# willSapgreen/stereo-vision

Measured on AMD Instinct MI355X. Metric: stereo pairs/sec (ELAS 1242x375, ROBOTICS, D1+D2+LR), higher is better.
Workload: dtype u8

## Files before the change

### include/svh.h

```cpp
#ifndef SVH_H
#define SVH_H

#include <stddef.h>
#include <stdint.h>

#ifdef __cplusplus
extern "C" {
#endif

#define SVH_OK                 0
#define SVH_ERR_FEW_SUPPORT    1
#define SVH_ERR_BAD_ARG       -1
#define SVH_ERR_HIP           -2
#define SVH_ERR_UNSUPPORTED   -3
#define SVH_ERR_NO_DEVICE     -4
#define SVH_ERR_BAD_DIMS      -7

typedef struct svh_elas_params {
    int32_t disp_min;
    int32_t disp_max;
    float   support_threshold;
    int32_t support_texture;
    int32_t candidate_stepsize;
    int32_t incon_window_size;
// ... 92 lines not shown
typedef struct svh_elas_stream svh_elas_stream;
svh_elas_stream* svh_elas_stream_open(svh_elas* e, const int32_t* dims, int32_t depth);
int32_t svh_elas_stream_push(svh_elas_stream* s, const uint8_t* I1, const uint8_t* I2,
                             float* D1, float* D2, uint64_t* ticket);
int32_t svh_elas_stream_push_device(svh_elas_stream* s, const uint8_t* dI1, const uint8_t* dI2,
                                    float* dD1, float* dD2, uint64_t* ticket);
int32_t svh_elas_stream_flush(svh_elas_stream* s);
int32_t svh_elas_stream_pop(svh_elas_stream* s, uint64_t* ticket, int32_t* status, int32_t timeout_ms);
int32_t svh_elas_stream_close(svh_elas_stream* s);
int32_t svh_elas_stream_push_device_n(svh_elas_stream* s, int32_t n, const uint8_t* dI1, const uint8_t* dI2,
                                      size_t in_stride, float* dD1, float* dD2, size_t out_stride,
                                      uint64_t* first_ticket);
int32_t svh_elas_stream_pop_n(svh_elas_stream* s, int32_t n, int32_t* status, int32_t* popped);
int32_t svh_elas_stream_push_n(svh_elas_stream* s, int32_t n, const uint8_t* const* I1, const uint8_t* const* I2,
                               float* const* D1, float* const* D2, uint64_t* first_ticket);

int64_t svh_elas_trim(void);

int32_t svh_elas_set_lanes(int32_t lanes);
int32_t svh_elas_set_group(int32_t pairs);

int32_t svh_elas_set_stage(int32_t where);
void svh_elas_stage_stats(int64_t* device_groups, int64_t* handed_back);
void svh_elas_get_settings(int32_t out[4]);

enum svh_elas_stage {
    SVH_ELAS_DESC1 = 0,
    SVH_ELAS_DESC2,
    SVH_ELAS_DCAN_RAW,
    SVH_ELAS_SUPPORT,
    SVH_ELAS_TRI1,
    SVH_ELAS_TRI2,
    SVH_ELAS_PLANES1,
    SVH_ELAS_PLANES2,
    SVH_ELAS_GRID1,
    SVH_ELAS_GRID2,
    SVH_ELAS_D1_RAW,
    SVH_ELAS_D2_RAW,
    SVH_ELAS_D1_LR,
    SVH_ELAS_D2_LR,
    SVH_ELAS_D1_SEG,
    SVH_ELAS_D2_SEG,
    SVH_ELAS_D1_GAP,
    SVH_ELAS_D2_GAP,
    SVH_ELAS_STAGE_COUNT
};
// ... 175 lines not shown
```

### stereo-vision_amd/csrc/elas_engine.cpp

```cpp
#include <hip/hip_runtime.h>
#include <stdio.h>
#include <string.h>

#include <atomic>
#include <chrono>
#include <condition_variable>
#include <deque>
#include <functional>
#include <algorithm>
#include <map>
#include <memory>
#include <mutex>
#include <string>
#include <thread>
#include <vector>

#include "hip_guard.h"
#include "svh_internal.h"

namespace svh {

static thread_local int t_device = 0;

#define HIP_TRY(kind, expr) SVH_HIP_TRY(nullptr, kind, expr)
// ... 72 lines not shown
    EventProfiler prof;
    int device = 0;
    hipStream_t stream = nullptr;
    hipEvent_t wait_ev = nullptr;
    hipStream_t copy_stream = nullptr;
    hipEvent_t match_ev = nullptr, copy_ev = nullptr;
    bool poll_wait = false;
    bool parallel_host = true;
    bool lone_group = true;
    int32_t W = 0, H = 0, disp_max = -1, step = 0, grid_size = 0, sub = -1, gcap = 0;
    Dims d{};
    bool desc_fly = false;
    int64_t owner_hi = 0;
    size_t prior_cap = 0;
    size_t ntri_max = 0;
    std::vector<HostPrior> hp;
    std::vector<int32_t> P;
    StageDev stg{};
    bool stage_ok = false;
    hipEvent_t stage_ev = nullptr;
    bool resident = false;
    bool force_host = false;
    float P_key[5] = {-1, -1, -1, -1, -1};
    size_t o_P = 0, o_sup = 0, o_tri = 0;

    void release() {
        if (!stream) return;
        (void)hipSetDevice(device);
        static_cast<LaneBufs&>(*this) = LaneBufs();
        stage_ok = false; stg = StageDev{};
        P_key[0] = -1;
        W = H = 0;
    }

    void destroy() {
        if (!stream) return;
        (void)hipSetDevice(device);
        release();
        for (hipEvent_t* e : {&wait_ev, &match_ev, &copy_ev, &stage_ev})
            if (*e) {
                (void)hipEventDestroy(*e);
                *e = nullptr;
            }
        for (hipEvent_t e : prof.ev) (void)hipEventDestroy(e);
        prof.ev.clear();
        prof.names.clear();
        if (copy_stream) (void)hipStreamDestroy(copy_stream);
        (void)hipStreamDestroy(stream);
        copy_stream = stream = nullptr;
    }

    int ensure(const svh_elas_params& p, int32_t w, int32_t h, int32_t g) {
        if (!stream) {
            HIP_TRY(none, hipSetDevice(device));
// ... 256 lines not shown
        if (!g_hostprof || !g_hp_pairs) return;
        static const char* nm[HP_N] = {"enqueue A", "waits", "filters", "delaunay", "pack", "enqueue B"};
        double tot = 0;
        for (int i = 0; i < HP_N; i++) tot += g_hp_ns[i];
        fprintf(stderr, "[svh host prof] %llu pairs, %.1f us cpu/pair:", (unsigned long long)g_hp_pairs.load(),
                tot / 1e3 / g_hp_pairs);
        for (int i = 0; i < HP_N; i++) fprintf(stderr, "  %s %.1f", nm[i], g_hp_ns[i] / 1e3 / g_hp_pairs);
        fprintf(stderr, "\n");
    }
};
static HostProfDump g_hp_dump;
#define HP_MARK(slot) do { if (g_hostprof) { uint64_t n_ = cpu_ns(); g_hp_ns[slot] += n_ - hp_t; hp_t = n_; } } while (0)

static int stage_mode_from_env() {
    const char* e = svh::env("SVH_STAGE");
    if (!e || !*e || !strcmp(e, "auto") || !strcmp(e, "-1")) return -1;
    if (!strcmp(e, "host") || !strcmp(e, "0")) return 0;
    if (!strcmp(e, "device") || !strcmp(e, "1")) return 1;
    fprintf(stderr, "svhip: SVH_STAGE=%s is not one of auto|-1, host|0, device|1: using auto\n", e);
    return -1;
}

static std::atomic<int64_t> g_stage_dev_groups{0}, g_stage_redo_groups{0};

static hipError_t event_wait(Lane& L, hipEvent_t ev) {
    if (!L.poll_wait || g_wait_us <= 0) return hipEventSynchronize(ev);
    for (;;) {
        hipError_t e = hipEventQuery(ev);
        if (e != hipErrorNotReady) return e;
        std::this_thread::sleep_for(std::chrono::microseconds(g_wait_us.load(std::memory_order_relaxed)));
    }
}

static int run_group_body(Lane& L, const svh_elas_params& p, const int32_t* dims, const GroupIO& io,
                          int32_t* status, Taps* taps, svh_elas* timing, int mode, int prefer_device);

static int run_group(Lane& L, const svh_elas_params& p, const int32_t* dims, const GroupIO& io,
                     int32_t* status, Taps* taps, svh_elas* timing, int mode = RG_ALL, int prefer_device = 0) {
    const int rc = run_group_body(L, p, dims, io, status, taps, timing, mode, prefer_device);
    if (rc == SVH_ERR_HIP) {
        const std::string keep = svh_last_error();
        if (L.stream) (void)hipStreamSynchronize(L.stream);
        if (L.copy_stream) (void)hipStreamSynchronize(L.copy_stream);
        (void)hipGetLastError();
        L.prof.used = 0;
        L.resident = false;
// ... 15 lines not shown
    if (rc) return rc;
    if (g > 1) taps = nullptr;
    const Dims& d = L.d;
    hipStream_t s = L.stream;
    L.prof.stream = s;
    const LaunchCtx cx = {s, g_prof_on.load() ? &L.prof : nullptr, L.lone_group};
    const size_t N = (size_t)W * H, DN = (size_t)d.DW * d.DH;
    const size_t nc = (size_t)d.Wc * d.Hc;
    const bool tapping = taps && taps->enabled;
    double t0 = now_ms();
    uint64_t hp_t = g_hostprof ? cpu_ns() : 0;

    GroupHdr* hdr = reinterpret_cast<GroupHdr*>(L.h_prior.p);
    DevMaps out;
    if (io.out_device) {
        out.D[0] = io.dD[0]; out.D[1] = io.dD[1]; out.stride[0] = out.stride[1] = io.out_stride;
    } else {
        out.D[0] = L.D; out.D[1] = L.D + DN; out.stride[0] = out.stride[1] = 2 * DN;
    }
    bool early_d2 = false;
    int32_t plane_radius = 2;

    auto enqueue_phase_b = [&](size_t o_P, size_t o_sup, size_t o_tri, int32_t total_sup, int32_t total_tri,
                               int32_t tri_bound) -> int {
        GroupDev G;
        G.hdr = reinterpret_cast<const GroupHdr*>(L.prior_dev.p);
        G.P = reinterpret_cast<const int32_t*>(L.prior_dev + o_P);
        G.support = reinterpret_cast<const int32_t*>(L.prior_dev + o_sup);
        G.tri = reinterpret_cast<const int32_t*>(L.prior_dev + o_tri);
        G.raster = L.raster;
        G.planes = L.planes;
        G.seed = L.seed;
        G.mask = L.mask;
        G.lists = L.lists;
        G.desc = L.desc;
        G.desc_fly = L.desc_fly ? 1 : 0;
        G.owner = L.owner;
        if (L.owner_hi + 1 + tri_bound >= INT32_MAX) {
            HIP_TRY(copy, hipMemsetAsync(L.owner, 0, (size_t)2 * L.gcap * N * sizeof(int32_t), s));
            L.owner_hi = 0;
        }
        G.owner_base = (int32_t)L.owner_hi;
        L.owner_hi += 1 + tri_bound;
        G.Draw = L.Draw;
        G.plane_radius = plane_radius;
        G.prior_absmax = 0;
        for (int32_t dd = 0; dd <= plane_radius && dd < (int32_t)L.P.size(); dd++)
            G.prior_absmax = std::max(G.prior_absmax, (int32_t)std::min<int64_t>(std::llabs((long long)L.P[dd]), INT32_MAX));
        launch_prior(cx, p, d, g, total_sup, total_tri, G);
        if (tapping) {
            const int32_t n1 = hdr->tri_end[0], n2 = hdr->tri_end[1] - hdr->tri_end[0];
            rc = tap_dev(L, taps, SVH_ELAS_PLANES1, L.planes.p, (size_t)6 * n1); if (rc) return rc;
            rc = tap_dev(L, taps, SVH_ELAS_PLANES2, L.planes.p + (size_t)6 * n1, (size_t)6 * n2); if (rc) return rc;
            const size_t words = (size_t)d.gw * d.gh * d.gwords;
            std::vector<uint32_t> m(2 * words);
            HIP_TRY(copy, hipMemcpyAsync(m.data(), L.mask, m.size() * sizeof(uint32_t), hipMemcpyDeviceToHost, s));
            HIP_TRY(wait, lane_wait(L));
            for (int k = 0; k < 2; k++) {
                std::vector<int32_t> gr;
                expand_grid(p, d, m.data() + k * words, gr);
                tap_host(taps, SVH_ELAS_GRID1 + k, gr.data(), gr.size());
            }
        }
        launch_owner(cx, p, d, g, total_tri, G);
        const bool tiles = !tapping && post_tiles_ok(p);
        const char* match_err = nullptr;
        const bool lr_done = launch_match(cx, p, d, g, G, &out, tapping, &match_err);
        if (match_err) return fail(SVH_ERR_HIP, std::string("launch_match: ") + match_err);
        early_d2 = !io.out_device && lr_done && !tapping && p.postprocess_only_left;
        if (early_d2) {
            if (!L.copy_stream) {
                HIP_TRY(none, hipStreamCreateWithFlags(&L.copy_stream, hipStreamNonBlocking));
                HIP_TRY(none, hipEventCreateWithFlags(&L.match_ev, hipEventDisableTiming));
                HIP_TRY(none, hipEventCreateWithFlags(&L.copy_ev, hipEventDisableTiming));
            }
            HIP_TRY(none, hipEventRecord(L.match_ev, s));
        }
        if (tapping) {
            rc = tap_dev(L, taps, SVH_ELAS_D1_RAW, L.Draw.p, DN); if (rc) return rc;
            rc = tap_dev(L, taps, SVH_ELAS_D2_RAW, L.Draw.p + DN, DN); if (rc) return rc;
        }
        const PostScratch ps = {L.tmp, L.labels, L.counts, L.seg_nroots};
        const int nside = p.postprocess_only_left ? 1 : 2;
        if (!lr_done) launch_lr(cx, p, d, g, G, out);
        if (tapping) {
            rc = tap_dev(L, taps, SVH_ELAS_D1_LR, out.D[0], DN); if (rc) return rc;
            rc = tap_dev(L, taps, SVH_ELAS_D2_LR, out.D[1], DN); if (rc) return rc;
// ... 42 lines not shown
            HIP_TRY(none, hipStreamWaitEvent(L.copy_stream, L.match_ev, 0));
            rc = copy_map(1, L.copy_stream, active);
            if (rc) return rc;
            HIP_TRY(none, hipEventRecord(L.copy_ev, L.copy_stream));
        }
        for (int k = 0; k < (early_d2 ? 1 : 2); k++) {
            rc = copy_map(k, s, active);
            if (rc) return rc;
        }
        if (early_d2) HIP_TRY(none, hipStreamWaitEvent(s, L.copy_ev, 0));
        return SVH_OK;
    };
    auto active_of = [&](int32_t j) {
        return L.h_counts.p->nsup[j] >= 3 && !(L.h_counts.p->flags[j] & (STG_DUP | STG_OVERFLOW));
    };

    auto finish = [&]() -> int {
        HIP_TRY(wait, lane_wait(L));
        HIP_TRY(launch, hipGetLastError());
        L.prof.collect();
        HP_MARK(HP_WAIT);
        if (!L.resident) return SVH_OK;
        g_stage_dev_groups++;
        bool redo = false;
        for (int32_t j = 0; j < g; j++) redo = redo || (L.h_counts.p->flags[j] & (STG_DUP | STG_OVERFLOW)) != 0;
        if (redo) {
            g_stage_redo_groups++;
            L.resident = false;
            L.force_host = true;
            rc = run_group(L, p, dims, io, status, taps, timing, RG_ALL, 0);
            L.force_host = false;
            return rc;
        }
        for (int32_t j = 0; j < g; j++) {
            if (L.h_counts.p->nsup[j] < 3) {
                printf("ERROR: Need at least 3 support points!\n");
                fflush(stdout);
                status[j] = SVH_ERR_FEW_SUPPORT;
            } else {
                status[j] = SVH_OK;
            }
        }
        return SVH_OK;
    };
    if (mode == RG_FINISH) return finish();

// ... 64 lines not shown
        L.resident = !L.force_host && L.stage_ok &&
                     (sm == 1 || (sm < 0 && prefer_device && stage_device_preferred(p, d, prefer_device > 1)));
        if (L.resident && prefer_device) L.poll_wait = true;
        if (!L.resident || tapping)
            HIP_TRY(copy, hipMemcpyAsync(L.h_dcan, L.dcan, g * nc * sizeof(int16_t), hipMemcpyDeviceToHost, s));
        if (L.resident) {
            prior_table(p, L.P, &plane_radius);
            const float key[5] = {p.beta, p.gamma, p.sigma, p.sradius, (float)p.disp_max};
            if (memcmp(key, L.P_key, sizeof(key)) != 0) {
                memcpy(L.h_prior + L.o_P, L.P.data(), L.P.size() * sizeof(int32_t));
                HIP_TRY(copy, hipMemcpyAsync(L.prior_dev + L.o_P, L.h_prior + L.o_P, L.P.size() * sizeof(int32_t),
                                       hipMemcpyHostToDevice, s));
                HIP_TRY(wait, hipStreamSynchronize(s));
                memcpy(L.P_key, key, sizeof(key));
            }
            if (tapping) {
                HIP_TRY(wait, hipStreamSynchronize(s));
                if (!L.desc_fly) {
                    rc = tap_dev(L, taps, SVH_ELAS_DESC1, L.desc.p, N * 16); if (rc) return rc;
                    rc = tap_dev(L, taps, SVH_ELAS_DESC2, L.desc.p + N * 16, N * 16); if (rc) return rc;
                }
                tap_host(taps, SVH_ELAS_DCAN_RAW, L.h_dcan.p, nc);
            }
            launch_stage_device(cx, p, d, g, L.stg, reinterpret_cast<GroupHdr*>(L.prior_dev.p),
                                reinterpret_cast<int32_t*>(L.prior_dev + L.o_sup),
                                reinterpret_cast<int32_t*>(L.prior_dev + L.o_tri));
            if (!L.stage_ev) HIP_TRY(none, hipEventCreateWithFlags(&L.stage_ev, hipEventDisableTiming));
            HIP_TRY(copy, hipMemcpyAsync(L.h_counts, L.stg.counts, sizeof(StageCounts), hipMemcpyDeviceToHost, s));
            HIP_TRY(none, hipEventRecord(L.stage_ev, s));
            if (tapping) {
                HIP_TRY(copy, hipMemcpyAsync(hdr, L.prior_dev, sizeof(GroupHdr), hipMemcpyDeviceToHost, s));
                HIP_TRY(wait, hipStreamSynchronize(s));
                if (hdr->active[0]) {
                    rc = tap_dev(L, taps, SVH_ELAS_SUPPORT, reinterpret_cast<int32_t*>(L.prior_dev + L.o_sup),
                                 (size_t)3 * hdr->total_sup); if (rc) return rc;
                    rc = tap_dev(L, taps, SVH_ELAS_TRI1, reinterpret_cast<int32_t*>(L.prior_dev + L.o_tri),
                                 (size_t)3 * hdr->tri_end[0]); if (rc) return rc;
                    rc = tap_dev(L, taps, SVH_ELAS_TRI2,
                                 reinterpret_cast<int32_t*>(L.prior_dev + L.o_tri) + (size_t)3 * hdr->tri_end[0],
                                 (size_t)3 * (hdr->tri_end[1] - hdr->tri_end[0])); if (rc) return rc;
                }
            }
            if (!tapping || hdr->active[0]) {
                const int32_t tri_bound = 2 * g * 2 * L.stg.sup_cap;
                rc = enqueue_phase_b(L.o_P, L.o_sup, L.o_tri, -1, -1, tri_bound);
                if (rc) return rc;
            }
        }
        HP_MARK(HP_ENQ_A);
    }
    if (!(mode & RG_HOST_B)) return SVH_OK;
    double t1 = t0, t2 = t0;
    if (L.resident) {
        if (!io.out_device) {
            HIP_TRY(wait, event_wait(L, L.stage_ev));
            HP_MARK(HP_WAIT);
            int32_t active[kMaxGroup];
            for (int32_t j = 0; j < g; j++) active[j] = active_of(j);
            rc = copy_out(active);
            if (rc) return rc;
        }
        if (g_hostprof) g_hp_pairs += g;
        HP_MARK(HP_ENQ_B);
        t1 = t2 = now_ms();
    } else {
    const bool warm = L.parallel_host && g == 1;
    if (warm) helpers_warm(3, 1500);
    struct WarmOff {
// ... 65 lines not shown
    const size_t o_sup = off;
    for (int32_t j = 0; j < g; j++) {
        const std::vector<int32_t>& v = L.hp[j].support;
        if (!v.empty()) memcpy(L.h_prior + off, v.data(), v.size() * sizeof(int32_t));
        off += v.size() * sizeof(int32_t);
    }
    off = (off + 63) & ~(size_t)63;
    const size_t o_tri = off;
    for (int32_t j = 0; j < g; j++)
        for (int k = 0; k < 2; k++) {
            const std::vector<int32_t>& v = L.hp[j].tri[k];
            if (!v.empty()) memcpy(L.h_prior + off, v.data(), v.size() * sizeof(int32_t));
            off += v.size() * sizeof(int32_t);
        }
    if (off > L.prior_cap) return fail(SVH_ERR_BAD_ARG, "prior exceeds staging capacity");
    if (warm_off.on) {
        helpers_warm(0, 0);
        warm_off.on = false;
    }
    t2 = now_ms();
    HP_MARK(HP_PACK);

    HIP_TRY(copy, hipMemcpyAsync(L.prior_dev, L.h_prior, off, hipMemcpyHostToDevice, s));
    rc = enqueue_phase_b(o_P, o_sup, o_tri, total_sup, total_tri, total_tri);
    if (rc) return rc;
    rc = copy_out(hdr->active);
    if (rc) return rc;
    HP_MARK(HP_ENQ_B);
    }
    if (!(mode & RG_FINISH)) return SVH_OK;
    rc = finish();
    if (rc) return rc;
    double t3 = now_ms();
    if (timing) {
        timing->tnames = {"Descriptor+Support Matches (device)", "Filters+Delaunay (host)",
                          "Planes+Grid+Matching+L/R+Segments+Gap+Mean (device)"};
        timing->tms = {(float)(t1 - t0), (float)(t2 - t1), (float)(t3 - t2)};
        if (L.resident) {
            timing->tnames = {"enqueue (host)", "whole pipeline incl. Filters+Delaunay (device)"};
            timing->tms = {(float)(t1 - t0), (float)(t3 - t1)};
        }
    }
    return SVH_OK;
}

}

// ... 698 lines not shown
    support_from_candidates(*p, d, dcan, s);
    const int32_t n = (int32_t)(s.size() / 3);
    for (int32_t i = 0; i < n && i < cap; i++)
        for (int k = 0; k < 3; k++) support[3 * i + k] = s[3 * i + k];
    return n;
}


int32_t svh_elas_set_stage(int32_t where) {
    g_stage_mode.store(where < 0 ? -1 : (where ? 1 : 0));
    return g_stage_mode.load();
}

void svh_debug_stage_stamps(int64_t* out32) {
    Pool* p = pool_for(t_device);
    std::lock_guard<std::mutex> lk(p->mu);
    for (Lane* l : p->lanes)
        if (l->stage_ok) {
            (void)hipMemcpy(out32, l->stg.counts->dbg, 32 * sizeof(int64_t), hipMemcpyDeviceToHost);
            return;
        }
}

void svh_elas_stage_stats(int64_t* device_groups, int64_t* handed_back) {
    if (device_groups) *device_groups = g_stage_dev_groups.load();
    if (handed_back) *handed_back = g_stage_redo_groups.load();
}

void svh_elas_get_settings(int32_t out[4]) {
    if (!out) return;
    out[0] = g_lanes.load();
    out[1] = g_group_set.load() ? g_group.load() : 0;
    out[2] = g_stage_mode.load();
    out[3] = g_wait_us;
}

int32_t svh_elas_set_group(int32_t pairs) {
    if (pairs < 1) pairs = 1;
    if (pairs > kMaxGroup) pairs = kMaxGroup;
    g_group.store(pairs);
    g_group_set.store(true);
    return pairs;
}

}
```

### stereo-vision_amd/csrc/elas_kernels.hip

```cpp
#include <hip/hip_runtime.h>

#include <algorithm>
#include <cstdlib>

#include "dev_common.h"
#include "svh_internal.h"

namespace svh {

namespace {

constexpr int kWave = 64;

template <int kCtrl, int kRowMask>
__device__ __forceinline__ uint32_t dpp_min_step(uint32_t v) {
    const uint32_t o =
        (uint32_t)__builtin_amdgcn_update_dpp((int)0xFFFFFFFFu, (int)v, kCtrl, kRowMask, 0xF, false);
    return o < v ? o : v;
}

__device__ __forceinline__ uint32_t wave_min_u32(uint32_t v) {
    v = dpp_min_step<0xB1, 0xF>(v);
    v = dpp_min_step<0x4E, 0xF>(v);
    v = dpp_min_step<0x141, 0xF>(v);
    v = dpp_min_step<0x140, 0xF>(v);
    v = dpp_min_step<0x142, 0xA>(v);
    v = dpp_min_step<0x143, 0xC>(v);
    return (uint32_t)__builtin_amdgcn_readlane((int)v, 63);
// ... 612 lines not shown
            if (mine >= 0) s_todo[base + __builtin_popcountll(mask & ((1ull << lane) - 1))] = (uint8_t)c;
            base += __builtin_popcountll(mask);
            if (c < ncand && mine < 0) dcan[c] = (int16_t)((uc0 + c) > 0 ? -1 : 0);
        }
        if (lane == 0) s_ntodo = base;
    }
    __syncthreads();
    const int ntodo = s_ntodo;
    for (int t0 = 4 * wave; t0 < ntodo; t0 += kPerRound) {
        const int t = t0 + grp;
        const bool have = t < ntodo;
        const int c = have ? (int)s_todo[t] : 0;
        const int d = have ? (int)s_fwd[c] : 0;
        const int uc = uc0 + c, u = uc * P.step;
        const int ub = have ? u - d : 5;
        const int t2 = !have ? 0 : kFly ? (int)s_texR[ub - xr0] : (int)texture16(d2[(size_t)v * P.W + ub]);
        const int dd = support_match_rows(R, L, t2, ub, true, have, P, gl);
        const int diff = d > dd ? d - dd : dd - d;
        const int out = (dd >= 0 && diff <= P.lr_threshold) ? d : -1;
        if (have && gl == 0) dcan[c] = (int16_t)out;
    }
}

__device__ bool solve3(double A[3][3], double B[3]) {
    bool used[3] = {false, false, false};
    for (int it = 0; it < 3; it++) {
        double big = 0.0;
        int pr = 0, pc = 0;
        for (int j = 0; j < 3; j++) {
            if (used[j]) continue;
            for (int k = 0; k < 3; k++)
                if (!used[k] && fabs(A[j][k]) >= big) {
                    big = fabs(A[j][k]);
                    pr = j;
                    pc = k;
                }
        }
        used[pc] = true;
        if (pr != pc) {
            for (int l = 0; l < 3; l++) {
                double t = A[pr][l];
                A[pr][l] = A[pc][l];
                A[pc][l] = t;
            }
            double t = B[pr];
            B[pr] = B[pc];
            B[pc] = t;
        }
        if (fabs(A[pc][pc]) < 1e-20) return false;
        const double inv = __ddiv_rn(1.0, A[pc][pc]);
        A[pc][pc] = 1.0;
        for (int l = 0; l < 3; l++) A[pc][l] = __dmul_rn(A[pc][l], inv);
        B[pc] = __dmul_rn(B[pc], inv);
        for (int r = 0; r < 3; r++) {
            if (r == pc) continue;
            const double f = A[r][pc];
            A[r][pc] = 0.0;
            for (int l = 0; l < 3; l++) A[r][l] = __dsub_rn(A[r][l], __dmul_rn(A[pc][l], f));
            B[r] = __dsub_rn(B[r], __dmul_rn(B[pc], f));
        }
    }
    return true;
}

__global__ __launch_bounds__(256) void k_prior(GroupDev G, int total_tri_arg) {
    const int total_tri = total_tri_arg >= 0 ? total_tri_arg : G.hdr->total_tri;
    for (int gid = blockIdx.x * 256 + threadIdx.x; (gid - (int)threadIdx.x) < 2 * total_tri; gid += gridDim.x * 256) {
    const int T = gid >> 1, rs = gid & 1;
    const bool live = T < total_tri;
    const int Tc = live ? T : 0;
    int first;
    const int slot = tri_slot(G.hdr, Tc, &first);
    const int pair = slot >> 1, side = slot & 1;
    const int32_t* sup = G.support + 3 * (size_t)G.hdr->sup_off[pair];
    const int32_t* c = G.tri + 3 * (size_t)Tc;
    int32_t su[3], sv[3], sd[3];
#pragma unroll
    for (int k = 0; k < 3; k++) {
        const int32_t* s = sup + 3 * c[k];
        su[k] = s[0];
        sv[k] = s[1];
        sd[k] = s[2];
    }
    float mine[3];
    {
        double A[3][3], B[3];
        for (int r = 0; r < 3; r++) {
            A[r][0] = (double)(rs ? su[r] - sd[r] : su[r]);
            A[r][1] = (double)sv[r];
            A[r][2] = 1.0;
            B[r] = (double)sd[r];
        }
        if (solve3(A, B)) {
            mine[0] = (float)B[0];
            mine[1] = (float)B[1];
            mine[2] = (float)B[2];
        } else {
            mine[0] = mine[1] = mine[2] = 0.f;
        }
    }
    float pl[6];
#pragma unroll
    for (int k = 0; k < 3; k++) {
        const float other = __shfl_xor(mine[k], 1);
        pl[k] = rs ? other : mine[k];
        pl[3 + k] = rs ? mine[k] : other;
    }
    if (!live || rs) continue;
#pragma unroll
    for (int k = 0; k < 6; k++) G.planes[6 * (size_t)T + k] = pl[k];

    float tu[3], tv[3];
#pragma unroll
    for (int k = 0; k < 3; k++) {
        tu[k] = side ? (float)(su[k] - sd[k]) : (float)su[k];
        tv[k] = (float)sv[k];
// ... 1645 lines not shown
                    const uint8_t* desc, int16_t* dcan, bool fly) {
    SupportParams P;
    P.W = d.W; P.H = d.H; P.Wc = d.Wc; P.Hc = d.Hc; P.step = d.step; P.npairs = g;
    P.disp_min = p.disp_min; P.disp_max = p.disp_max;
    P.support_texture = p.support_texture; P.lr_threshold = p.lr_threshold;
    P.support_threshold = p.support_threshold;
    size_t lds = 0;
    const int sb = support_strip(p, d, &lds);
    if (sb) {
        Timed timed_(cx, "k_support");
        const int chunks = (d.Wc + sb - 1) / sb;
        const dim3 grid((unsigned)(((d.Hc * g + 7) / 8) * 8 * chunks), 1, 1);
        hipStream_t st = (hipStream_t)cx.stream;
        if (sb == 32 && fly) hipLaunchKernelGGL((k_support_lds<32, 512, true>), grid, dim3(512), lds, st, desc, dcan, P);
        else if (sb == 32) hipLaunchKernelGGL((k_support_lds<32, 512, false>), grid, dim3(512), lds, st, desc, dcan, P);
        else if (fly) hipLaunchKernelGGL((k_support_lds<64, 512, true>), grid, dim3(512), lds, st, desc, dcan, P);
        else hipLaunchKernelGGL((k_support_lds<64, 512, false>), grid, dim3(512), lds, st, desc, dcan, P);
    } else {
        const int cands = d.Wc * d.Hc;
        LAUNCH("k_support", k_support, dim3((cands + 3) / 4, g), dim3(256), desc, dcan, P);
    }
}

void launch_prior(const LaunchCtx& cx, const svh_elas_params& p, const Dims& d, int32_t g,
                  int32_t total_sup, int32_t total_tri, const GroupDev& G) {
    hipStream_t s = (hipStream_t)cx.stream;
    const int cells = d.gw * d.gh;
    const size_t words = (size_t)2 * g * cells * d.gwords;
    (void)hipMemsetAsync(G.seed, 0, words * sizeof(uint32_t), s);
    const int sup_bound = std::max(256, g * d.Wc * d.Hc / 6), tri_bound = 4 * sup_bound;
    const int nt = total_tri >= 0 ? total_tri : tri_bound, ns = total_sup >= 0 ? total_sup : sup_bound;
    if (nt > 0) LAUNCH("k_prior", k_prior, dim3((2 * nt + 255) / 256), dim3(256), G, total_tri);
    if (ns > 0)
        LAUNCH("k_grid_seed", k_grid_seed, dim3((ns + 255) / 256), dim3(256), G, total_sup,
               d.gw, d.gh, d.gwords, p.grid_size, p.disp_max);
    LAUNCH("k_grid_dilate", k_grid_dilate, dim3((unsigned)((words + 255) / 256)), dim3(256), G,
           2 * g, d.gw, d.gh, d.gwords);
    if (d.gwords <= 8 && G.lists)
        LAUNCH("k_grid_list", k_grid_list, dim3((unsigned)((2 * g * cells + 3) / 4)), dim3(256), G, 2 * g * cells,
               d.gwords);
}

void launch_owner(const LaunchCtx& cx, const svh_elas_params& p, const Dims& d, int32_t g,
                  int32_t total_tri, const GroupDev& G) {
    if (total_tri == 0) return;
    const int nt = total_tri >= 0 ? total_tri : 4 * std::max(256, g * d.Wc * d.Hc / 6);
    const bool wide = (double)d.H * ((double)d.W + 2.0 * p.disp_max) > 4194304.0;
    const int fix_all = svh::env("SVH_OWNER_FIX_ALL") ? atoi(svh::env("SVH_OWNER_FIX_ALL")) : (wide ? 1 : 0);
    const dim3 go(xcd_blocks((nt + 3) / 4));
    LAUNCH("k_owner", k_owner<false>, go, dim3(256), G, total_tri, d.W, d.H,
           p.subsampling, 0);
    LAUNCH("k_owner_fix", k_owner<true>, go, dim3(256), G, total_tri, d.W, d.H,
           p.subsampling, fix_all);
}

static bool match_list_usable(const svh_elas_params& p, const Dims& d, int32_t prior_absmax, int32_t plane_radius,
                              bool have_lists, MatchList* Qout, size_t* lds_out) {
    static const bool ordered = svh::env("SVH_MATCH_ORDERED") != nullptr;
    const bool keyed_ok = !ordered && prior_absmax < (1 << 19) && p.disp_max < 512 && plane_radius <= 15 &&
                          d.W < 65536 && p.grid_size > 1;
    static const bool list_off = svh::env("SVH_MATCH_LIST") && atoi(svh::env("SVH_MATCH_LIST")) == 0;
    static const bool list_sub = !(svh::env("SVH_MATCH_LIST_SUB") && atoi(svh::env("SVH_MATCH_LIST_SUB")) == 0);
    if (!(keyed_ok && !list_off && (!p.subsampling || list_sub) && d.gwords <= 8 && have_lists && prior_absmax < 28000 &&
          d.DW <= 8 * 256))
        return false;
    MatchList Q;
    Q.Wr = (d.W + 7) / 8 * 8;
    Q.Ws = ((d.W + 3) & ~3) + 2;
    static const bool wide768 = !(svh::env("SVH_MATCH_WIDE768") && atoi(svh::env("SVH_MATCH_WIDE768")) == 0);
// ... 497 lines not shown
```

### stereo-vision_amd/csrc/elas_stage_kernels.hip

```cpp
#include <hip/hip_runtime.h>

#include <mutex>

#include <algorithm>

#include "dev_common.h"
#include "svh_internal.h"
#include "dt_core.h"

namespace svh {

namespace {

constexpr int16_t kInv = -32768;

struct LatticeParams {
    int W, H, Wc, Hc, step, ws, thr, need, add_corners, sup_cap;
};

__device__ __forceinline__ void lattice_consistency_events(int16_t* val, uint32_t* cntw, int32_t* wl, int nc,
                                                           const LatticeParams& P, int* s_n) {
    const int tid = threadIdx.x, Wc = P.Wc, Hc = P.Hc;
    int32_t* alive = wl;
    int32_t* fresh[2] = {wl + nc, wl + 2 * (size_t)nc};
// ... 592 lines not shown
            __syncthreads();
        }
    }
    if (remap) {
        for (int t = 2 * m - 1 + tid; t < 2 * m_all - 1; t += kT)
            *reinterpret_cast<int4*>(mg.ids + 4 * (size_t)t) = make_int4(-1, -1, -1, 0);
        __syncthreads();
    }
    const MeshG& mesh = mg;
    const int nrec = 2 * m - 1;
    int live = 0;
    for (int t = 1 + tid; t < nrec; t += kT) {
        const int4 v = *reinterpret_cast<const int4*>(mesh.ids + 4 * (size_t)t);
        live += (v.x >= 0) & (v.y >= 0) & (v.z >= 0);
    }
    int tot;
    block_exclusive_scan<kT>(live, s_scan, &tot);
    if (tid == 0) S.counts->ntri[slot] = tot;
    STAMP(30);
#undef STAMP
}

__global__ __launch_bounds__(256) void k_stage_pack(StageDev S, DtParams P, int g, GroupHdr* hdr, int32_t* support,
                                                    int32_t* tri) {
    __shared__ int s_scan[256 / 64 + 1];
    const int slot = blockIdx.x, pair = slot >> 1, side = slot & 1, tid = threadIdx.x;
    int sup_off = 0, tri_off = 0, total_sup = 0, total_tri = 0;
    bool active_me = false;
    for (int j = 0; j < g; j++) {
        const bool act = S.counts->nsup[j] >= 3 && !(S.counts->flags[j] & (STG_DUP | STG_OVERFLOW));
        const int ns = act ? S.counts->nsup[j] : 0;
        if (j < pair) sup_off += ns;
        if (j == pair) active_me = act;
        total_sup += ns;
        for (int k = 0; k < 2; k++) {
            const int nt = act ? S.counts->ntri[2 * j + k] : 0;
            if (2 * j + k < slot) tri_off += nt;
            total_tri += nt;
        }
    }
    if (slot == 0 && tid == 0) {
        hdr->npairs = g;
        int so = 0, te = 0;
        for (int j = 0; j < g; j++) {
            const bool act = S.counts->nsup[j] >= 3 && !(S.counts->flags[j] & (STG_DUP | STG_OVERFLOW));
            hdr->active[j] = act ? 1 : 0;
            hdr->sup_off[j] = so;
            so += act ? S.counts->nsup[j] : 0;
            for (int k = 0; k < 2; k++) {
// ... 77 lines not shown
    static const size_t kb = svh::env("SVH_DT_LDS_KB") ? (size_t)atoi(svh::env("SVH_DT_LDS_KB")) : 96;
    return std::min<size_t>(159, std::max<size_t>(kb, 8));
}
static size_t dt_lds_bytes(const svh_elas_params& p, const Dims& d, bool big) {
    const size_t hist = 4 * (size_t)(2 * (dt_columns(p, d) + d.H) + 2);
    if (big) return std::max<size_t>(hist, 159 * 1024);
    size_t want = dt_small_kb() * 1024;
    if (want > 63 * 1024 && !dt_lds_optin(false, dt_small_kb() * 1024)) want = 63 * 1024;
    return std::max<size_t>(hist, want);
}

bool stage_device_ok(const svh_elas_params& p, const Dims& d) {
    const int wx = dt_columns(p, d);
    return 4 * (size_t)(2 * (wx + d.H) + 2) <= 63 * 1024 && wx < (1 << 14) && d.H < (1 << 14);
}

bool stage_device_preferred(const svh_elas_params& p, const Dims& d, bool deep_batch) {
    const size_t nc = (size_t)d.Wc * d.Hc;
    if (!stage_device_ok(p, d)) return false;
    return deep_batch || 2 * ((nc + 1) & ~(size_t)1) + 4 * ((nc + 3) / 4) <= 62 * 1024;
}

void launch_stage_device(const LaunchCtx& cx, const svh_elas_params& p, const Dims& d, int32_t g, const StageDev& S,
                         GroupHdr* hdr, int32_t* support, int32_t* tri) {
    hipStream_t s = (hipStream_t)cx.stream;
    LatticeParams L;
    L.W = d.W; L.H = d.H; L.Wc = d.Wc; L.Hc = d.Hc; L.step = d.step;
    L.ws = p.incon_window_size; L.thr = p.incon_threshold; L.need = p.incon_min_support;
    L.add_corners = p.add_corners; L.sup_cap = S.sup_cap;
    const size_t nc = (size_t)d.Wc * d.Hc;
    const size_t lat_bytes = 2 * ((nc + 1) & ~(size_t)1) + 4 * ((nc + 3) / 4);
    if (L.need > 0 && (2 * L.ws + 1) * (2 * L.ws + 1) <= 255 && L.need <= 255) {
        Timed t(cx, "k_lattice_count");
        hipLaunchKernelGGL(k_lattice_count, dim3((d.Wc + LCX - 1) / LCX, (d.Hc + LCY - 1) / LCY, g), dim3(64, 4), 0, s,
                           S, L);
    }
    {
        Timed t(cx, "k_lattice");
        if (lat_bytes <= 62 * 1024)
            hipLaunchKernelGGL(k_lattice<true>, dim3(g), dim3(512), lat_bytes, s, S, L);
        else
            hipLaunchKernelGGL(k_lattice<false>, dim3(g), dim3(512), 0, s, S, L);
    }
    DtParams D;
    D.W = dt_columns(p, d); D.H = d.H; D.sup_cap = S.sup_cap; D.rec_cap = S.rec_cap;
    D.xoff = std::max(p.disp_max, 0);
    const bool big = dt_large(d) && dt_lds_optin(true, 159 * 1024);
// ... 2 lines not shown
    static const int dt_uniform = svh::env("SVH_DT_UNIFORM") ? atoi(svh::env("SVH_DT_UNIFORM")) : -1;
    D.uniform = dt_uniform >= 0 ? dt_uniform : (cx.latency && !big ? 1 : 0);
    const size_t dt_lds = dt_lds_bytes(p, d, big);
    D.lds_ints = (int)(dt_lds / 4);
    D.lds_cap = (int)std::min<size_t>((dt_lds - 32) / 48 - 1, 8000);
    {
        Timed t(cx, "k_delaunay");
        if (big && dt_split()) {
            hipLaunchKernelGGL((k_delaunay<1024, 1>), dim3(2 * g), dim3(1024), dt_lds, s, S, D);
            DtParams B = D;
            B.lds_ints = 0;
            B.lds_cap = 0;
            hipLaunchKernelGGL((k_delaunay<1024, 2>), dim3(2 * g), dim3(1024), 0, s, S, B);
        } else if (big) {
            hipLaunchKernelGGL((k_delaunay<1024, 0>), dim3(2 * g), dim3(1024), dt_lds, s, S, D);
        } else {
            if (dt_small_threads() == 1024) hipLaunchKernelGGL((k_delaunay<1024, 0>), dim3(2 * g), dim3(1024), dt_lds, s, S, D);
            else if (dt_small_threads() == 512) hipLaunchKernelGGL((k_delaunay<512, 0>), dim3(2 * g), dim3(512), dt_lds, s, S, D);
            else hipLaunchKernelGGL((k_delaunay<256, 0>), dim3(2 * g), dim3(256), dt_lds, s, S, D);
        }
    }
    {
        Timed t(cx, "k_stage_pack");
        hipLaunchKernelGGL(k_stage_pack, dim3(2 * g), dim3(256), 0, s, S, D, g, hdr, support, tri);
    }
}

}
```

### stereo-vision_amd/csrc/svh_internal.h

```cpp
#ifndef SVH_INTERNAL_H
#define SVH_INTERNAL_H

#include <stddef.h>
#include <stdint.h>

#include <functional>
#include <vector>

#include "../../include/svh.h"
#include "svh_config.h"

namespace svh {

struct Dims {
    int32_t W, H;
    int32_t DW, DH;
    int32_t step;
    int32_t Wc, Hc;
    int32_t gw, gh;
    int32_t gwords;
};
Dims make_dims(const svh_elas_params& p, int32_t W, int32_t H);

constexpr int kMaxGroup = 32;
// ... 87 lines not shown
    size_t stride[2];
};

struct GroupDev {
    const GroupHdr* hdr;
    const int32_t* support;
    const int32_t* tri;
    const int32_t* P;
    TriRaster* raster;
    float* planes;
    uint32_t* seed;
    uint32_t* mask;
    uint16_t* lists;
    const uint8_t* desc;
    int32_t* owner;
    float* Draw;
    int32_t plane_radius;
    int32_t owner_base;
    int32_t prior_absmax;
    int32_t desc_fly;
};

void launch_stage_device(const LaunchCtx& cx, const svh_elas_params& p, const Dims& d, int32_t g,
                         const StageDev& S, GroupHdr* hdr, int32_t* support, int32_t* tri);

void launch_descriptor(const LaunchCtx& cx, const DevImages& img, int32_t g, int32_t W, int32_t H,
                       int32_t half, uint8_t* desc, bool fly);
bool descriptors_on_the_fly(const svh_elas_params& p, const Dims& d, int32_t prior_absmax, int32_t plane_radius,
                            bool have_lists);
void launch_support(const LaunchCtx& cx, const svh_elas_params& p, const Dims& d, int32_t g,
                    const uint8_t* desc, int16_t* dcan, bool fly);
void launch_prior(const LaunchCtx& cx, const svh_elas_params& p, const Dims& d, int32_t g,
                  int32_t total_sup, int32_t total_tri, const GroupDev& G);
void launch_owner(const LaunchCtx& cx, const svh_elas_params& p, const Dims& d, int32_t g,
                  int32_t total_tri, const GroupDev& G);
bool launch_match(const LaunchCtx& cx, const svh_elas_params& p, const Dims& d, int32_t g,
                  const GroupDev& G, const DevMaps* lr_out, bool write_raw, const char** error);
void launch_lr(const LaunchCtx& cx, const svh_elas_params& p, const Dims& d, int32_t g,
               const GroupDev& G, const DevMaps& out);
struct PostScratch {
    float* tmp;
    int32_t* labels;
    int32_t* counts;
    int32_t* nroots;
};
bool post_tiles_ok(const svh_elas_params& p);
void launch_gap_mean_tiles(const LaunchCtx& cx, const svh_elas_params& p, const Dims& d, int32_t g,
                           int32_t nside, const GroupDev& G, const DevMaps& out, const PostScratch& S);
void launch_segments(const LaunchCtx& cx, const svh_elas_params& p, const Dims& d, int32_t g,
                     int32_t nside, const GroupDev& G, const DevMaps& out, const PostScratch& s, bool mask = true);
void launch_gap(const LaunchCtx& cx, const svh_elas_params& p, const Dims& d, int32_t g,
                int32_t nside, const GroupDev& G, const DevMaps& out, const PostScratch& s);
void launch_adaptive_mean(const LaunchCtx& cx, const svh_elas_params& p, const Dims& d, int32_t g,
                          int32_t nside, const GroupDev& G, const DevMaps& out, const PostScratch& s);
void launch_median(const LaunchCtx& cx, const Dims& d, int32_t g, int32_t nside, const GroupDev& G,
                   const DevMaps& out, const PostScratch& s);
void launch_segments_label(const LaunchCtx& cx, const svh_elas_params& p, const Dims& d, int32_t g,
                           int32_t nside, const GroupDev& G, const DevMaps& in, const PostScratch& s);
// ... 4 lines not shown
```

Baseline: 33040.

## Size phase-B launches from recent history and fold seed clear and count readback into pack kernel

Each lane keeps a short history of the support and triangle counts from recent device-staged groups. It uses the maximum of that history plus a margin to size the k_prior, k_grid_seed and k_owner grids, instead of always launching for the worst-case bound. The seed-buffer memset and the device-to-host copy of StageCounts are moved into k_stage_pack, which zeroes the seed buffer and writes the counts directly to host memory, removing two queued blit operations. The 3x3 pivoting solver in k_prior is also replaced with a branch-free, unrolled version. Risks: under-sized grids when the count jumps past the history margin, which grid-stride loops should absorb but which is tracked with shortfall counters. A kernel writing into pinned host memory may also carry different visibility or latency costs.

After: 33690, median of 6. 1.02x the previous value.

```diff
diff --git a/include/svh.h b/include/svh.h
--- a/include/svh.h
+++ b/include/svh.h
@@ -138,6 +138,7 @@
 
 int32_t svh_elas_set_stage(int32_t where);
 void svh_elas_stage_stats(int64_t* device_groups, int64_t* handed_back);
+void svh_elas_sizing_stats(int64_t* out4);
 void svh_elas_get_settings(int32_t out[4]);
 
 enum svh_elas_stage {
diff --git a/stereo-vision_amd/csrc/elas_engine.cpp b/stereo-vision_amd/csrc/elas_engine.cpp
--- a/stereo-vision_amd/csrc/elas_engine.cpp
+++ b/stereo-vision_amd/csrc/elas_engine.cpp
@@ -118,6 +118,12 @@
     bool resident = false;
     bool force_host = false;
     float P_key[5] = {-1, -1, -1, -1, -1};
+    static constexpr int kHist = 4;
+    int32_t hist_sup[kHist] = {}, hist_tri[kHist] = {};
+    int hist_n = 0, hist_at = 0;
+    int32_t hist_g = 0;
+    svh_elas_params hist_p{};
+    PhaseBSize sized{};
     size_t o_P = 0, o_sup = 0, o_tri = 0;
 
     void release() {
@@ -126,6 +132,7 @@
         static_cast<LaneBufs&>(*this) = LaneBufs();
         stage_ok = false; stg = StageDev{};
         P_key[0] = -1;
+        hist_n = 0;
         W = H = 0;
     }
 
@@ -428,6 +435,7 @@
 }
 
 static std::atomic<int64_t> g_stage_dev_groups{0}, g_stage_redo_groups{0};
+static std::atomic<int64_t> g_sized_bound{0}, g_sized_hist{0}, g_short_tri{0}, g_short_sup{0};
 
 static hipError_t event_wait(Lane& L, hipEvent_t ev) {
     if (!L.poll_wait || g_wait_us <= 0) return hipEventSynchronize(ev);
@@ -489,7 +497,7 @@
     int32_t plane_radius = 2;
 
     auto enqueue_phase_b = [&](size_t o_P, size_t o_sup, size_t o_tri, int32_t total_sup, int32_t total_tri,
-                               int32_t tri_bound) -> int {
+                               int32_t tri_bound, const PhaseBSize& size) -> int {
         GroupDev G;
         G.hdr = reinterpret_cast<const GroupHdr*>(L.prior_dev.p);
         G.P = reinterpret_cast<const int32_t*>(L.prior_dev + o_P);
@@ -514,7 +522,7 @@
         G.prior_absmax = 0;
         for (int32_t dd = 0; dd <= plane_radius && dd < (int32_t)L.P.size(); dd++)
             G.prior_absmax = std::max(G.prior_absmax, (int32_t)std::min<int64_t>(std::llabs((long long)L.P[dd]), INT32_MAX));
-        launch_prior(cx, p, d, g, total_sup, total_tri, G);
+        launch_prior(cx, p, d, g, total_sup, total_tri, G, size);
         if (tapping) {
             const int32_t n1 = hdr->tri_end[0], n2 = hdr->tri_end[1] - hdr->tri_end[0];
             rc = tap_dev(L, taps, SVH_ELAS_PLANES1, L.planes.p, (size_t)6 * n1); if (rc) return rc;
@@ -529,7 +537,7 @@
                 tap_host(taps, SVH_ELAS_GRID1 + k, gr.data(), gr.size());
             }
         }
-        launch_owner(cx, p, d, g, total_tri, G);
+        launch_owner(cx, p, d, g, total_tri, G, size);
         const bool tiles = !tapping && post_tiles_ok(p);
         const char* match_err = nullptr;
         const bool lr_done = launch_match(cx, p, d, g, G, &out, tapping, &match_err);
@@ -618,6 +626,29 @@
         HP_MARK(HP_WAIT);
         if (!L.resident) return SVH_OK;
         g_stage_dev_groups++;
+        {
+            int32_t ts = 0, tt = 0;
+            for (int32_t j = 0; j < g; j++)
+                if (active_of(j)) {
+                    ts += L.h_counts.p->nsup[j];
+                    tt += L.h_counts.p->ntri[2 * j] + L.h_counts.p->ntri[2 * j + 1];
+                }
+            if (L.hist_n && (L.hist_g != g || memcmp(&L.hist_p, &p, sizeof(p)) != 0)) L.hist_n = 0;
+            if (!L.hist_n) L.hist_at = 0;
+            L.hist_g = g;
+            L.hist_p = p;
+            L.hist_sup[L.hist_at] = ts;
+            L.hist_tri[L.hist_at] = tt;
+            L.hist_at = (L.hist_at + 1) % Lane::kHist;
+            L.hist_n = std::min(L.hist_n + 1, (int)Lane::kHist);
+            if (L.sized.from_history) {
+                g_sized_hist++;
+                if (tt > L.sized.nt) g_short_tri++;
+                if (ts > L.sized.ns) g_short_sup++;
+            } else {
+                g_sized_bound++;
+            }
+        }
         bool redo = false;
         for (int32_t j = 0; j < g; j++) redo = redo || (L.h_counts.p->flags[j] & (STG_DUP | STG_OVERFLOW)) != 0;
         if (redo) {
@@ -728,11 +759,14 @@
                 }
                 tap_host(taps, SVH_ELAS_DCAN_RAW, L.h_dcan.p, nc);
             }
+            const bool blits = svh::env("SVH_STAGE_BLITS") && atoi(svh::env("SVH_STAGE_BLITS")) != 0;
             launch_stage_device(cx, p, d, g, L.stg, reinterpret_cast<GroupHdr*>(L.prior_dev.p),
                                 reinterpret_cast<int32_t*>(L.prior_dev + L.o_sup),
-                                reinterpret_cast<int32_t*>(L.prior_dev + L.o_tri));
+                                reinterpret_cast<int32_t*>(L.prior_dev + L.o_tri),
+                                blits ? nullptr : L.seed.p, (size_t)2 * g * d.gw * d.gh * d.gwords,
+                                blits ? nullptr : L.h_counts.p);
             if (!L.stage_ev) HIP_TRY(none, hipEventCreateWithFlags(&L.stage_ev, hipEventDisableTiming));
-            HIP_TRY(copy, hipMemcpyAsync(L.h_counts, L.stg.counts, sizeof(StageCounts), hipMemcpyDeviceToHost, s));
+            if (blits) HIP_TRY(copy, hipMemcpyAsync(L.h_counts, L.stg.counts, sizeof(StageCounts), hipMemcpyDeviceToHost, s));
             HIP_TRY(none, hipEventRecord(L.stage_ev, s));
             if (tapping) {
                 HIP_TRY(copy, hipMemcpyAsync(hdr, L.prior_dev, sizeof(GroupHdr), hipMemcpyDeviceToHost, s));
@@ -747,9 +781,19 @@
                                  (size_t)3 * (hdr->tri_end[1] - hdr->tri_end[0])); if (rc) return rc;
                 }
             }
+            L.sized = PhaseBSize{};
             if (!tapping || hdr->active[0]) {
                 const int32_t tri_bound = 2 * g * 2 * L.stg.sup_cap;
-                rc = enqueue_phase_b(L.o_P, L.o_sup, L.o_tri, -1, -1, tri_bound);
+                int32_t hint_sup = 0, hint_tri = 0;
+                const bool use_hist = !(svh::env("SVH_PHASEB_HISTORY") && atoi(svh::env("SVH_PHASEB_HISTORY")) == 0);
+                if (use_hist && L.hist_n && L.hist_g == g && memcmp(&L.hist_p, &p, sizeof(p)) == 0)
+                    for (int k = 0; k < L.hist_n; k++) {
+                        hint_sup = std::max(hint_sup, L.hist_sup[k]);
+                        hint_tri = std::max(hint_tri, L.hist_tri[k]);
+                    }
+                L.sized = phase_b_size(d, g, -1, -1, hint_sup, hint_tri);
+                L.sized.seed_cleared = !blits;
+                rc = enqueue_phase_b(L.o_P, L.o_sup, L.o_tri, -1, -1, tri_bound, L.sized);
                 if (rc) return rc;
             }
         }
@@ -861,7 +905,7 @@
     HP_MARK(HP_PACK);
 
     HIP_TRY(copy, hipMemcpyAsync(L.prior_dev, L.h_prior, off, hipMemcpyHostToDevice, s));
-    rc = enqueue_phase_b(o_P, o_sup, o_tri, total_sup, total_tri, total_tri);
+    rc = enqueue_phase_b(o_P, o_sup, o_tri, total_sup, total_tri, total_tri, phase_b_size(d, g, total_sup, total_tri, 0, 0));
     if (rc) return rc;
     rc = copy_out(hdr->active);
     if (rc) return rc;
@@ -1606,6 +1650,14 @@
         }
 }
 
+void svh_elas_sizing_stats(int64_t* out4) {
+    if (!out4) return;
+    out4[0] = svh::g_sized_bound.load();
+    out4[1] = svh::g_sized_hist.load();
+    out4[2] = svh::g_short_tri.load();
+    out4[3] = svh::g_short_sup.load();
+}
+
 void svh_elas_stage_stats(int64_t* device_groups, int64_t* handed_back) {
     if (device_groups) *device_groups = g_stage_dev_groups.load();
     if (handed_back) *handed_back = g_stage_redo_groups.load();
diff --git a/stereo-vision_amd/csrc/elas_kernels.hip b/stereo-vision_amd/csrc/elas_kernels.hip
--- a/stereo-vision_amd/csrc/elas_kernels.hip
+++ b/stereo-vision_amd/csrc/elas_kernels.hip
@@ -4,6 +4,7 @@
 #include <cstdlib>
 
 #include "dev_common.h"
+#include "prior_core.h"
 #include "svh_internal.h"
 
 namespace svh {
@@ -662,47 +663,6 @@
     }
 }
 
-__device__ bool solve3(double A[3][3], double B[3]) {
-    bool used[3] = {false, false, false};
-    for (int it = 0; it < 3; it++) {
-        double big = 0.0;
-        int pr = 0, pc = 0;
-        for (int j = 0; j < 3; j++) {
-            if (used[j]) continue;
-            for (int k = 0; k < 3; k++)
-                if (!used[k] && fabs(A[j][k]) >= big) {
-                    big = fabs(A[j][k]);
-                    pr = j;
-                    pc = k;
-                }
-        }
-        used[pc] = true;
-        if (pr != pc) {
-            for (int l = 0; l < 3; l++) {
-                double t = A[pr][l];
-                A[pr][l] = A[pc][l];
-                A[pc][l] = t;
-            }
-            double t = B[pr];
-            B[pr] = B[pc];
-            B[pc] = t;
-        }
-        if (fabs(A[pc][pc]) < 1e-20) return false;
-        const double inv = __ddiv_rn(1.0, A[pc][pc]);
-        A[pc][pc] = 1.0;
-        for (int l = 0; l < 3; l++) A[pc][l] = __dmul_rn(A[pc][l], inv);
-        B[pc] = __dmul_rn(B[pc], inv);
-        for (int r = 0; r < 3; r++) {
-            if (r == pc) continue;
-            const double f = A[r][pc];
-            A[r][pc] = 0.0;
-            for (int l = 0; l < 3; l++) A[r][l] = __dsub_rn(A[r][l], __dmul_rn(A[pc][l], f));
-            B[r] = __dsub_rn(B[r], __dmul_rn(B[pc], f));
-        }
-    }
-    return true;
-}
-
 __global__ __launch_bounds__(256) void k_prior(GroupDev G, int total_tri_arg) {
     const int total_tri = total_tri_arg >= 0 ? total_tri_arg : G.hdr->total_tri;
     for (int gid = blockIdx.x * 256 + threadIdx.x; (gid - (int)threadIdx.x) < 2 * total_tri; gid += gridDim.x * 256) {
@@ -725,13 +685,14 @@
     float mine[3];
     {
         double A[3][3], B[3];
+#pragma unroll
         for (int r = 0; r < 3; r++) {
             A[r][0] = (double)(rs ? su[r] - sd[r] : su[r]);
             A[r][1] = (double)sv[r];
             A[r][2] = 1.0;
             B[r] = (double)sd[r];
         }
-        if (solve3(A, B)) {
+        if (prior::solve3(A, B)) {
             mine[0] = (float)B[0];
             mine[1] = (float)B[1];
             mine[2] = (float)B[2];
@@ -2423,14 +2384,23 @@
     }
 }
 
+PhaseBSize phase_b_size(const Dims& d, int32_t g, int32_t total_sup, int32_t total_tri, int32_t hint_sup, int32_t hint_tri) {
+    const int sup_bound = std::max(256, g * d.Wc * d.Hc / 6), tri_bound = 4 * sup_bound;
+    PhaseBSize z;
+    z.from_history = total_tri < 0 && total_sup < 0 && hint_sup > 0 && hint_tri > 0;
+    z.ns = total_sup >= 0 ? total_sup : z.from_history ? std::min(sup_bound, hint_sup + hint_sup / 8 + 1) : sup_bound;
+    z.nt = total_tri >= 0 ? total_tri : z.from_history ? std::min(tri_bound, hint_tri + hint_tri / 8 + 1) : tri_bound;
+    z.seed_cleared = false;
+    return z;
+}
+
 void launch_prior(const LaunchCtx& cx, const svh_elas_params& p, const Dims& d, int32_t g,
-                  int32_t total_sup, int32_t total_tri, const GroupDev& G) {
+                  int32_t total_sup, int32_t total_tri, const GroupDev& G, const PhaseBSize& size) {
     hipStream_t s = (hipStream_t)cx.stream;
     const int cells = d.gw * d.gh;
     const size_t words = (size_t)2 * g * cells * d.gwords;
-    (void)hipMemsetAsync(G.seed, 0, words * sizeof(uint32_t), s);
-    const int sup_bound = std::max(256, g * d.Wc * d.Hc / 6), tri_bound = 4 * sup_bound;
-    const int nt = total_tri >= 0 ? total_tri : tri_bound, ns = total_sup >= 0 ? total_sup : sup_bound;
+    if (!size.seed_cleared) (void)hipMemsetAsync(G.seed, 0, words * sizeof(uint32_t), s);
+    const int nt = size.nt, ns = size.ns;
     if (nt > 0) LAUNCH("k_prior", k_prior, dim3((2 * nt + 255) / 256), dim3(256), G, total_tri);
     if (ns > 0)
         LAUNCH("k_grid_seed", k_grid_seed, dim3((ns + 255) / 256), dim3(256), G, total_sup,
@@ -2443,9 +2413,9 @@
 }
 
 void launch_owner(const LaunchCtx& cx, const svh_elas_params& p, const Dims& d, int32_t g,
-                  int32_t total_tri, const GroupDev& G) {
+                  int32_t total_tri, const GroupDev& G, const PhaseBSize& size) {
     if (total_tri == 0) return;
-    const int nt = total_tri >= 0 ? total_tri : 4 * std::max(256, g * d.Wc * d.Hc / 6);
+    const int nt = size.nt;
     const bool wide = (double)d.H * ((double)d.W + 2.0 * p.disp_max) > 4194304.0;
     const int fix_all = svh::env("SVH_OWNER_FIX_ALL") ? atoi(svh::env("SVH_OWNER_FIX_ALL")) : (wide ? 1 : 0);
     const dim3 go(xcd_blocks((nt + 3) / 4));
diff --git a/stereo-vision_amd/csrc/elas_stage_kernels.hip b/stereo-vision_amd/csrc/elas_stage_kernels.hip
--- a/stereo-vision_amd/csrc/elas_stage_kernels.hip
+++ b/stereo-vision_amd/csrc/elas_stage_kernels.hip
@@ -638,9 +638,22 @@
 }
 
 __global__ __launch_bounds__(256) void k_stage_pack(StageDev S, DtParams P, int g, GroupHdr* hdr, int32_t* support,
-                                                    int32_t* tri) {
+                                                    int32_t* tri, uint32_t* seed, size_t seed_words,
+                                                    StageCounts* h_counts) {
     __shared__ int s_scan[256 / 64 + 1];
     const int slot = blockIdx.x, pair = slot >> 1, side = slot & 1, tid = threadIdx.x;
+    if (seed) {
+        const size_t quads = seed_words / 4;
+        uint4* q = reinterpret_cast<uint4*>(seed);
+        for (size_t i = (size_t)blockIdx.x * 256 + tid; i < quads; i += (size_t)gridDim.x * 256) q[i] = make_uint4(0, 0, 0, 0);
+        for (size_t i = 4 * quads + (size_t)blockIdx.x * 256 + tid; i < seed_words; i += (size_t)gridDim.x * 256) seed[i] = 0;
+    }
+    if (h_counts && slot == 0) {
+        static_assert(sizeof(StageCounts) % 4 == 0, "copied word by word");
+        const uint32_t* src = reinterpret_cast<const uint32_t*>(S.counts);
+        uint32_t* dst = reinterpret_cast<uint32_t*>(h_counts);
+        for (int i = tid; i < (int)(sizeof(StageCounts) / 4); i += 256) dst[i] = src[i];
+    }
     int sup_off = 0, tri_off = 0, total_sup = 0, total_tri = 0;
     bool active_me = false;
     for (int j = 0; j < g; j++) {
@@ -764,7 +777,8 @@
 }
 
 void launch_stage_device(const LaunchCtx& cx, const svh_elas_params& p, const Dims& d, int32_t g, const StageDev& S,
-                         GroupHdr* hdr, int32_t* support, int32_t* tri) {
+                         GroupHdr* hdr, int32_t* support, int32_t* tri, uint32_t* seed, size_t seed_words,
+                         StageCounts* h_counts) {
     hipStream_t s = (hipStream_t)cx.stream;
     LatticeParams L;
     L.W = d.W; L.H = d.H; L.Wc = d.Wc; L.Hc = d.Hc; L.step = d.step;
@@ -813,8 +827,9 @@
     }
     {
         Timed t(cx, "k_stage_pack");
-        hipLaunchKernelGGL(k_stage_pack, dim3(2 * g), dim3(256), 0, s, S, D, g, hdr, support, tri);
-    }
-}
-
-}
+        hipLaunchKernelGGL(k_stage_pack, dim3(2 * g), dim3(256), 0, s, S, D, g, hdr, support, tri, seed,
+                           seed_words, h_counts);
+    }
+}
+
+}
diff --git a/stereo-vision_amd/csrc/prior_core.h b/stereo-vision_amd/csrc/prior_core.h
--- /dev/null
+++ b/stereo-vision_amd/csrc/prior_core.h
@@ -0,0 +1,106 @@
+#pragma once
+#include <math.h>
+#include "mono_core.h"
+
+namespace svh {
+namespace prior {
+
+MC_FN double pick3(int i, double a0, double a1, double a2) { return i == 0 ? a0 : i == 1 ? a1 : a2; }
+
+MC_FN bool solve3(const double A[3][3], double B[3]) {
+    const double B0 = B[0], B1 = B[1], B2 = B[2];
+    double big = 0.0;
+    int pr = 0, pc = 0;
+    for (int j = 0; j < 3; j++)
+        for (int k = 0; k < 3; k++) {
+            const double a = fabs(A[j][k]);
+            const bool ge = a >= big;
+            big = ge ? a : big;
+            pr = ge ? j : pr;
+            pc = ge ? k : pc;
+        }
+    double c[3], x[3], y[3];
+    for (int j = 0; j < 3; j++) {
+        const double a0 = A[j][0], a1 = A[j][1], a2 = A[j][2];
+        c[j] = pick3(pc, a0, a1, a2);
+        x[j] = pc == 0 ? a1 : a0;
+        y[j] = pc == 2 ? a1 : a2;
+    }
+    const double c0 = c[0], c1_ = c[1], c2 = c[2], x0 = x[0], x1 = x[1], x2 = x[2], y0 = y[0], y1 = y[1], y2 = y[2];
+    const double Pc = pick3(pr, c0, c1_, c2);
+    double Px = pick3(pr, x0, x1, x2);
+    double Py = pick3(pr, y0, y1, y2);
+    double Pb = pick3(pr, B0, B1, B2);
+    const double Qc = pick3(pc, c0, c1_, c2);
+    const double Qx = pick3(pc, x0, x1, x2);
+    const double Qy = pick3(pc, y0, y1, y2);
+    const double Qb = pick3(pc, B0, B1, B2);
+    const int lo = pc == 0 ? 1 : 0, hi = pc == 2 ? 1 : 2;
+    const bool lo_q = lo == pr, hi_q = hi == pr;
+    double m[2][2], f[2], b[2];
+    f[0] = lo_q ? Qc : (pc == 0 ? c1_ : c0);
+    m[0][0] = lo_q ? Qx : (pc == 0 ? x1 : x0);
+    m[0][1] = lo_q ? Qy : (pc == 0 ? y1 : y0);
+    b[0] = lo_q ? Qb : (pc == 0 ? B1 : B0);
+    f[1] = hi_q ? Qc : (pc == 2 ? c1_ : c2);
+    m[1][0] = hi_q ? Qx : (pc == 2 ? x1 : x2);
+    m[1][1] = hi_q ? Qy : (pc == 2 ? y1 : y2);
+    b[1] = hi_q ? Qb : (pc == 2 ? B1 : B2);
+    bool ok = !(fabs(Pc) < 1e-20);
+    {
+        const double inv = 1.0 / Pc;
+        Px = Px * inv;
+        Py = Py * inv;
+        Pb = Pb * inv;
+        for (int r = 0; r < 2; r++) {
+            m[r][0] = m[r][0] - Px * f[r];
+            m[r][1] = m[r][1] - Py * f[r];
+            b[r] = b[r] - Pb * f[r];
+        }
+    }
+    big = 0.0;
+    int qr = 0, qc = 0;
+    for (int j = 0; j < 2; j++)
+        for (int k = 0; k < 2; k++) {
+            const double a = fabs(m[j][k]);
+            const bool ge = a >= big;
+            big = ge ? a : big;
+            qr = ge ? j : qr;
+            qc = ge ? k : qc;
+        }
+    const bool r1 = qr == 1, c1 = qc == 1;
+    const double m00 = m[0][0], m01 = m[0][1], m10 = m[1][0], m11 = m[1][1], b0 = b[0], b1 = b[1];
+    const double Rp = r1 ? (c1 ? m11 : m10) : (c1 ? m01 : m00);
+    double Rz = r1 ? (c1 ? m10 : m11) : (c1 ? m00 : m01);
+    double Rb = r1 ? b1 : b0;
+    const double Sp = r1 ? (c1 ? m01 : m00) : (c1 ? m11 : m10);
+    double Sz = r1 ? (c1 ? m00 : m01) : (c1 ? m10 : m11);
+    double Sb = r1 ? b0 : b1;
+    const double Pp = c1 ? Py : Px;
+    double Pz = c1 ? Px : Py;
+    ok = ok && !(fabs(Rp) < 1e-20);
+    {
+        const double inv = 1.0 / Rp;
+        Rz = Rz * inv;
+        Rb = Rb * inv;
+        Pz = Pz - Rz * Pp;
+        Pb = Pb - Rb * Pp;
+        Sz = Sz - Rz * Sp;
+        Sb = Sb - Rb * Sp;
+    }
+    ok = ok && !(fabs(Sz) < 1e-20);
+    {
+        const double inv = 1.0 / Sz;
+        Sb = Sb * inv;
+        Pb = Pb - Sb * Pz;
+        Rb = Rb - Sb * Rz;
+    }
+    const double blo = c1 ? Sb : Rb, bhi = c1 ? Rb : Sb;
+    B[0] = pc == 0 ? Pb : blo;
+    B[1] = pc == 1 ? Pb : (pc == 0 ? blo : bhi);
+    B[2] = pc == 2 ? Pb : bhi;
+    return ok;
+}
+
+}
+}
diff --git a/stereo-vision_amd/csrc/svh_internal.h b/stereo-vision_amd/csrc/svh_internal.h
--- a/stereo-vision_amd/csrc/svh_internal.h
+++ b/stereo-vision_amd/csrc/svh_internal.h
@@ -133,7 +133,8 @@
 };
 
 void launch_stage_device(const LaunchCtx& cx, const svh_elas_params& p, const Dims& d, int32_t g,
-                         const StageDev& S, GroupHdr* hdr, int32_t* support, int32_t* tri);
+                         const StageDev& S, GroupHdr* hdr, int32_t* support, int32_t* tri,
+                         uint32_t* seed, size_t seed_words, StageCounts* h_counts);
 
 void launch_descriptor(const LaunchCtx& cx, const DevImages& img, int32_t g, int32_t W, int32_t H,
                        int32_t half, uint8_t* desc, bool fly);
@@ -141,10 +142,16 @@
                             bool have_lists);
 void launch_support(const LaunchCtx& cx, const svh_elas_params& p, const Dims& d, int32_t g,
                     const uint8_t* desc, int16_t* dcan, bool fly);
+struct PhaseBSize {
+    int32_t ns, nt;
+    bool from_history;
+    bool seed_cleared;
+};
+PhaseBSize phase_b_size(const Dims& d, int32_t g, int32_t total_sup, int32_t total_tri, int32_t hint_sup, int32_t hint_tri);
 void launch_prior(const LaunchCtx& cx, const svh_elas_params& p, const Dims& d, int32_t g,
-                  int32_t total_sup, int32_t total_tri, const GroupDev& G);
+                  int32_t total_sup, int32_t total_tri, const GroupDev& G, const PhaseBSize& size);
 void launch_owner(const LaunchCtx& cx, const svh_elas_params& p, const Dims& d, int32_t g,
-                  int32_t total_tri, const GroupDev& G);
+                  int32_t total_tri, const GroupDev& G, const PhaseBSize& size);
 bool launch_match(const LaunchCtx& cx, const svh_elas_params& p, const Dims& d, int32_t g,
                   const GroupDev& G, const DevMaps* lr_out, bool write_raw, const char** error);
 void launch_lr(const LaunchCtx& cx, const svh_elas_params& p, const Dims& d, int32_t g,
```
